# torchkge-team/torchkge

Measured on AMD Instinct MI355X. Metric: link-prediction triples scored/sec (filtered LP eval, both sides), higher is better.
Workload: dtype f32 (f16 hi/lo-split MFMA prefilter + exact f32 recheck; ranks bit-identical to f32)

## Files before the change

### torchkge_amd/csrc/lp_split_mfma.hip

```cpp
#include "kge_common.h"
#ifndef KGE_BUILD_NO_SLP
#error "build with -fno-slp-vectorize -DKGE_BUILD_NO_SLP=1 (torchkge_amd/csrc/build.py): SLP-packed v_pk_fma_f32 with a lane-crossing op_sel misreads beside co-executing MFMAs (profiles/r06/slp_bisect.txt)"
#endif

typedef _Float16 f16x8 __attribute__((ext_vector_type(8)));
typedef float f32x2 __attribute__((ext_vector_type(2)));
typedef float f32x16 __attribute__((ext_vector_type(16)));

namespace {

constexpr int TQ = 192, TC = 256;
constexpr int NT = 3;
constexpr int E_STAGE_BYTES = TC * 128;
constexpr int Q_STAGE_BYTES = TQ * 128;
constexpr int STAGE_BYTES = E_STAGE_BYTES + Q_STAGE_BYTES;
constexpr int UNC_CAP = 2048;
constexpr int GSETS = 4;
constexpr int SMEM_BYTES = 2 * STAGE_BYTES + 16 + UNC_CAP * 4 + TQ * 20 + TQ * GSETS * 12 + 16;
constexpr int SPLIT_SCALE_LOG2 = 12;

struct SplitParams {
    const char *Es, *Qs;
    int row_bytes;
    int units;
// ... 1871 lines not shown
                int qp_next, ct_next;
                item_qp_ct(it + 1, qp_next, ct_next);
                const int64_t next_q0 = (int64_t)qp_next * TQ;
                if (next_q0 != cur_q0) {
                    flush_counts(cur_q0);
                    cur_q0 = next_q0;
                    load_panel(cur_q0);
                }
            }
        }
        if (DBG && tl) {
            tsv[15] = __builtin_readcyclecounter();
            if (lane == 0) {
                unsigned long long *o = reinterpret_cast<unsigned long long *>(p.list) + ((wid >> 2) * KGE_TL_STAGES + g) * 16;
#pragma unroll
                for (int i = 0; i < 16; ++i) o[i] = tsv[i];
            }
        }
        if (++s == S) { s = 0; ++it; }
    }
#undef KGE_TS
#undef KGE_SMMA_PA
#undef KGE_SMMA_P
#undef KGE_HLOAD
#undef KGE_HWAIT
#undef KGE_SLOAD
#undef KGE_SWAIT
#undef KGE_DSR
    flush_counts(cur_q0);
}

template <bool VEC4>
__global__ __launch_bounds__(64, 2) void split_recheck_kernel(const kge_lp_desc d, const float *__restrict__ s_true,
                                                           const int32_t *__restrict__ list, int32_t cap,
                                                           const int32_t *__restrict__ list_count, int32_t *raw_count,
                                                           float *list_stat)
{
    __shared__ __attribute__((aligned(16))) float qs[64 * KGE_PS_LD];
    __shared__ __attribute__((aligned(16))) float es[64 * KGE_PS_LD];
    const int lane = threadIdx.x;
    const int n = (int)min((unsigned)*list_count, (unsigned)cap);
    if (list_stat && blockIdx.x == 0 && lane == 0) atomicAdd(list_stat, (float)n);
    const int ngroups = (n + 63) >> 6;
    for (int grp = blockIdx.x; grp < ngroups; grp += gridDim.x) {
        const int pi = grp * 64 + lane;
        const bool valid = pi < n;
        const int pj = valid ? pi : grp * 64;
        const int qi = list[2 * pj], ci = list[2 * pj + 1];
        const float sc = lp_pair_score_staged<VEC4>(d, qi, ci, qs, es);
        if (valid && !(sc >= s_true[qi])) atomicSub(&raw_count[qi], 1);
    }
}

__device__ __forceinline__ float recheck_e_segment(const float *__restrict__ T, int64_t ldt, int K, int ci,
                                                   const float *__restrict__ qrow, float *es, float acc)
{
    const int lane = threadIdx.x & 63;
    int k0 = 0;
    if (K >= KGE_PS_KC) {
        float4 e0, e1, e2, e3, e4, e5, e6, e7;
#define KGE_RR_FETCH(IT, KK)                                                                                  \
    {                                                                                                         \
        const int idx_ = lane + 64 * IT, rr_ = idx_ >> 3, pc_ = idx_ & 7;                                     \
        const int rc_ = __shfl(ci, rr_, 64);                                                                  \
        e##IT = *reinterpret_cast<const float4 *>(T + (int64_t)rc_ * ldt + (KK) + pc_ * 4);                   \
    }
#define KGE_RR_STORE(IT)                                                                                      \
    {                                                                                                         \
        const int idx_ = lane + 64 * IT, rr_ = idx_ >> 3, pc_ = idx_ & 7;                                     \
        *reinterpret_cast<float4 *>(es + rr_ * KGE_PS_LD + pc_ * 4) = e##IT;                                  \
    }
#define KGE_RR_ALL(M, ...) M(0, ##__VA_ARGS__) M(1, ##__VA_ARGS__) M(2, ##__VA_ARGS__) M(3, ##__VA_ARGS__) \
                           M(4, ##__VA_ARGS__) M(5, ##__VA_ARGS__) M(6, ##__VA_ARGS__) M(7, ##__VA_ARGS__)
        KGE_RR_ALL(KGE_RR_FETCH, 0)
        for (; k0 + KGE_PS_KC <= K; k0 += KGE_PS_KC) {
            KGE_RR_ALL(KGE_RR_STORE)
            if (k0 + 2 * KGE_PS_KC <= K) { KGE_RR_ALL(KGE_RR_FETCH, k0 + KGE_PS_KC) }
            __builtin_amdgcn_fence(__ATOMIC_SEQ_CST, "wavefront");
            acc = lp_chain_dot(qrow + k0, es + lane * KGE_PS_LD, KGE_PS_KC, acc);
            __builtin_amdgcn_fence(__ATOMIC_SEQ_CST, "wavefront");
        }
#undef KGE_RR_ALL
#undef KGE_RR_STORE
#undef KGE_RR_FETCH
    }
    for (; k0 < K; k0 += KGE_PS_KC) {
        const int kc = min(KGE_PS_KC, K - k0);
        const int pieces = kc >> 2;
        for (int idx = lane; idx < 64 * pieces; idx += 64) {
            const int rr = idx / pieces, pc = idx - rr * pieces;
            const int rc = __shfl(ci, rr, 64);
            *reinterpret_cast<float4 *>(es + rr * KGE_PS_LD + pc * 4) =
                *reinterpret_cast<const float4 *>(T + (int64_t)rc * ldt + k0 + pc * 4);
        }
        __builtin_amdgcn_fence(__ATOMIC_SEQ_CST, "wavefront");
        acc = lp_chain_dot(qrow + k0, es + lane * KGE_PS_LD, kc, acc);
        __builtin_amdgcn_fence(__ATOMIC_SEQ_CST, "wavefront");
    }
    return acc;
}

constexpr int RR_ROWS = 32, RR_PANEL = 96;

constexpr int RR_G = 4;

template <int NWV>
__global__ __launch_bounds__(64 * NWV) void split_recheck_regions_kernel(const kge_lp_desc d, const float *__restrict__ s_true,
                                                                        const int32_t *__restrict__ list, int32_t region_cap,
                                                                        const int32_t *__restrict__ region_count, int n_regions,
                                                                        int ldq, int seg_cols, int32_t *raw_count, float *list_stat,
                                                                        int32_t *list_count)
{
    extern __shared__ __attribute__((aligned(16))) float rr_smem[];
    const int tid = threadIdx.x, lane = tid & 63, wv = tid >> 6;
    float *qrows = rr_smem;
    float *es = rr_smem + RR_ROWS * ldq + wv * 64 * KGE_PS_LD;
    const int K = d.K0 + d.K1;
    int n_block = 0;
    auto stage = [&](int64_t q0, int c0, int c1) {
        const int np = (c1 - c0) >> 2;
        for (int idx = tid; idx < RR_ROWS * np; idx += 64 * NWV) {
            const int rr = idx / np, pc = idx - rr * np;
            const int64_t q = min(q0 + rr, d.B - 1);
            const int col = c0 + pc * 4;
            const float4 v = col < d.K0 ? *reinterpret_cast<const float4 *>(d.A0 + q * d.lda0 + col)
                                        : *reinterpret_cast<const float4 *>(d.A1 + q * d.lda1 + (col - d.K0));
            *reinterpret_cast<float4 *>(qrows + rr * ldq + pc * 4) = v;
        }
    };
    auto chain = [&](float acc, int ci, const float *qrow, int c0, int c1) -> float {
        if (c0 < d.K0) acc = recheck_e_segment(d.T0 + c0, d.ldt0, min(c1, d.K0) - c0, ci, qrow, es, acc);
        if (c1 > d.K0 && d.K1 > 0) {
            const int s0 = max(c0, d.K0);
            acc = recheck_e_segment(d.T1 + (s0 - d.K0), d.ldt1, c1 - s0, ci, qrow + (s0 - c0), es, acc);
        }
        return acc;
    };
    for (int reg = blockIdx.x; reg < n_regions; reg += gridDim.x) {
        const int n = (int)min((unsigned)region_count[reg], (unsigned)region_cap);
        if (n == 0) continue;
        n_block += n;
        const int64_t q0 = (int64_t)(reg / 3) * RR_PANEL + (reg % 3) * RR_ROWS;
        const int2 *ent = reinterpret_cast<const int2 *>(list) + (int64_t)reg * region_cap;
        if (K <= seg_cols) {
            __syncthreads();
            stage(q0, 0, K);
            __syncthreads();
            for (int c0 = wv * 64; c0 < n; c0 += NWV * 64) {
                const int pi = c0 + lane;
                const bool valid = pi < n;
                const int2 e = ent[valid ? pi : c0];
                const int qi = e.x, ci = e.y;
                const float acc = chain(0.0f, ci, qrows + (int)(qi - q0) * ldq, 0, K);
                const float sc = lp_epilogue_any(d, acc, qi, ci);
                if (valid && !(sc >= s_true[qi])) atomicSub(&raw_count[qi], 1);
            }
            continue;
        }
        for (int b0 = 0; b0 < n; b0 += NWV * 64 * RR_G) {
            float acc[RR_G];
            int qi[RR_G], ci[RR_G];
#pragma unroll
            for (int g = 0; g < RR_G; ++g) {
                const int c0 = b0 + (g * NWV + wv) * 64;
                const int pi = c0 + lane;
                const int2 e = ent[min(pi < n ? pi : c0, n - 1)];
                qi[g] = e.x; ci[g] = e.y; acc[g] = 0.0f;
            }
            for (int c0 = 0; c0 < K; c0 += seg_cols) {
                const int c1 = min(K, c0 + seg_cols);
                __syncthreads();
                stage(q0, c0, c1);
                __syncthreads();
#pragma unroll
                for (int g = 0; g < RR_G; ++g)
                    if (b0 + (g * NWV + wv) * 64 < n)
                        acc[g] = chain(acc[g], ci[g], qrows + (int)(qi[g] - q0) * ldq, c0, c1);
            }
#pragma unroll
            for (int g = 0; g < RR_G; ++g) {
                const int pi = b0 + (g * NWV + wv) * 64 + lane;
                if (pi < n) {
                    const float sc = lp_epilogue_any(d, acc[g], qi[g], ci[g]);
                    if (!(sc >= s_true[qi[g]])) atomicSub(&raw_count[qi[g]], 1);
                }
            }
        }
    }
    if (tid == 0 && n_block > 0) {
        if (list_stat) atomicAdd(list_stat, (float)n_block);
        if (list_count) atomicAdd(list_count, n_block);
    }
}

template <int NWAVES, bool DBG, int PM, int GS = 0, int LV = 0>
int launch_split(const SplitParams &p, int grid, hipStream_t s)
{
    auto k = lp_split_count_kernel<NWAVES, DBG, PM, GS, LV>;
    static int attr_dev[16];
    if (int e = kge_ensure_dyn_smem(reinterpret_cast<const void *>(k), SMEM_BYTES, attr_dev)) return e;
    hipLaunchKernelGGL(k, dim3(grid), dim3(64 * NWAVES), SMEM_BYTES, s, p);
    KGE_CHECK_LAUNCH();
    return 0;
}

int split_num_cus()
{
    static int n = 0;
    if (n == 0) {
        int dev = 0;
        hipDeviceProp_t prop;
        if (hipGetDevice(&dev) == hipSuccess && hipGetDeviceProperties(&prop, dev) == hipSuccess)
            n = prop.multiProcessorCount;
        if (n <= 0) n = 256;
    }
    return n;
}

inline int64_t round_up(int64_t x, int64_t m) { return (x + m - 1) / m * m; }

}

extern "C" int kge_lp_split_units(int K, int with_aug)
{
    return (int)round_up((K + (with_aug ? 1 : 0) + 15) / 16, 2);
}

extern "C" int64_t kge_lp_split_rows_padded(int64_t rows, int is_query) { return round_up(rows, is_query ? TQ : TC); }

extern "C" int kge_lp_split_rows(const float *X0, int64_t ld0, int K0, const float *X1, int64_t ld1, int K1,
                                 int64_t rows, int is_query, int aug_mode, const float *aug, float aug_mul,
                                 const float *norm2max0, const float *norm2max1, void *out, float *cell_ss,
                                 const int64_t *row_index, kge_stream_t stream)
{
    if (rows < 0 || K0 <= 0 || K1 < 0 || ld0 < K0 || (K1 > 0 && ld1 < K1) || aug_mode < 0 || aug_mode > 4)
        return KGE_EINVAL;
    if (rows == 0 && is_query) return 0;
    if ((rows > 0 && !X0) || (rows > 0 && K1 > 0 && !X1) || !out || ((aug_mode == 1 || aug_mode == 3) && rows > 0 && !aug))
        return KGE_EINVAL;
    SplitRowsParams p;
    p.X0 = X0; p.X1 = X1; p.ld0 = ld0; p.ld1 = ld1; p.K0 = K0; p.K1 = K1;
    p.rows = rows;
    p.rows_p = kge_lp_split_rows_padded(rows, is_query);
    p.aug_mode = aug_mode; p.aug = aug; p.aug_mul = aug_mul;
// ... 329 lines not shown
    int rc = kge_lp_desc_check(d);
    if (rc) return rc;
    if (d->B == 0 || d->N == 0) return 0;
    if (!s_true || !list || cap <= 0 || !list_count || !raw_count) return KGE_EINVAL;
    if (!KGE_LP_IS_MFMA(d->mode)) return KGE_EINVAL;
    const bool vec4 = kge_lp_vec4(*d);
    const int grid = split_num_cus() * kge_env_int("KGE_SPLIT_RECHECK_WAVES", 160 * 1024 / (2 * 64 * KGE_PS_LD * 4));
    if (vec4)
        hipLaunchKernelGGL(split_recheck_kernel<true>, dim3(grid), dim3(64), 0, kge_s(stream), *d, s_true, list, cap,
                           list_count, raw_count, list_stat);
    else
        hipLaunchKernelGGL(split_recheck_kernel<false>, dim3(grid), dim3(64), 0, kge_s(stream), *d, s_true, list,
                           cap, list_count, raw_count, list_stat);
    KGE_CHECK_LAUNCH();
    return 0;
}

extern "C" int kge_lp_split_regions(int64_t B)
{
    return (int)(kge_lp_split_rows_padded(B, 1) / RR_PANEL) * 3;
}

static int region_seg_cols(int K)
{
    const int max_ld = kge_env_int("KGE_REGION_MAX_BYTES", 36 * 1024) / (RR_ROWS * 4);
    const int ld_full = K + (((K >> 2) & 1) ? 0 : 4);
    if (ld_full <= max_ld) return K;
    const int seg_ld = min(max_ld, kge_env_int("KGE_REGION_SEG_BYTES", 20 * 1024) / (RR_ROWS * 4));
    int seg = ((seg_ld - 4) / 32) * 32;
    return seg < 32 ? 32 : seg;
}

extern "C" int kge_lp_split_regions_supported(const kge_lp_desc *d)
{
    if (kge_lp_desc_check(d) || !KGE_LP_IS_MFMA(d->mode) || !kge_lp_vec4(*d)) return 0;
    const int K = d->K0 + d->K1;
    if ((K + 2 + 15) / 16 > 32) return 0;
    if (region_seg_cols(K) < K && kge_env_int("KGE_REGION_SEGMENTS", 1) == 0) return 0;
    return 1;
}

extern "C" int kge_lp_split_recheck_regions(const kge_lp_desc *d, const float *s_true, const int32_t *list, int32_t cap,
                                            const int32_t *region_count, int32_t *raw_count, float *list_stat,
                                            int32_t *list_count, kge_stream_t stream)
{
    int rc = kge_lp_desc_check(d);
    if (rc) return rc;
    if (d->B == 0 || d->N == 0) return 0;
    if (!s_true || !list || cap <= 0 || !region_count || !raw_count) return KGE_EINVAL;
    if (!kge_lp_split_regions_supported(d)) return KGE_EINVAL;
    const int n_regions = kge_lp_split_regions(d->B);
    const int32_t region_cap = cap / n_regions;
    if (region_cap <= 0) return KGE_EINVAL;
    const int K = d->K0 + d->K1;
    const int seg = region_seg_cols(K);
    const int ldq = seg + (((seg >> 2) & 1) ? 0 : 4);
    const int nwv = kge_env_int("KGE_RECHECK_REGION_WAVES", 2);
    const int smem = (RR_ROWS * ldq + (nwv == 4 ? 4 : 2) * 64 * KGE_PS_LD) * 4;
    const int want = split_num_cus() * 6;
    const int grid = n_regions < want ? n_regions : want;
    static int attr2[16], attr4[16];
    if (nwv == 4) {
        auto k = split_recheck_regions_kernel<4>;
        if (int e = kge_ensure_dyn_smem(reinterpret_cast<const void *>(k), smem, attr4)) return e;
        hipLaunchKernelGGL(k, dim3(grid), dim3(256), smem, kge_s(stream), *d, s_true, list, region_cap, region_count, n_regions,
                           ldq, seg, raw_count, list_stat, list_count);
    } else {
        auto k = split_recheck_regions_kernel<2>;
        if (int e = kge_ensure_dyn_smem(reinterpret_cast<const void *>(k), smem, attr2)) return e;
        hipLaunchKernelGGL(k, dim3(grid), dim3(128), smem, kge_s(stream), *d, s_true, list, region_cap, region_count, n_regions,
                           ldq, seg, raw_count, list_stat, list_count);
    }
    KGE_CHECK_LAUNCH();
    return 0;
}

extern "C" int kge_absmax(const float *x, int64_t n, float *max_io, kge_stream_t stream)
{
    if (n < 0 || !max_io) return KGE_EINVAL;
    if (n == 0) return 0;
    if (!x) return KGE_EINVAL;
    const int64_t want = (n + 1023) / 1024;
    const int grid = (int)(want < 1024 ? want : 1024);
    hipLaunchKernelGGL(absmax_kernel, dim3(grid), dim3(256), 0, kge_s(stream), x, n, max_io);
    KGE_CHECK_LAUNCH();
    return 0;
}


extern "C" int kge_mfma_f16_selftest(void)
{
    constexpr int NT_ = 8;
    float ab[NT_][32], c[NT_], expect[NT_];
    for (int t = 0; t < NT_; ++t) { for (int k = 0; k < 32; ++k) ab[t][k] = 0.f; c[t] = 0.f; }
    auto A = [&](int t, int k) -> float & { return ab[t][k]; };
    auto Bv = [&](int t, int k) -> float & { return ab[t][16 + k]; };
    for (int k = 0; k < 16; ++k) { A(0, k) = 1.f; Bv(0, k) = 1.f; } A(0, 0) = 4096.f; Bv(0, 0) = 4096.f; expect[0] = 16777232.f;
    A(1, 0) = A(1, 1) = A(1, 2) = 1.f; Bv(1, 0) = Bv(1, 1) = Bv(1, 2) = 1.f; c[1] = 16777216.f; expect[1] = 16777220.f;
    A(2, 0) = 1.f; Bv(2, 0) = 1.f; c[2] = 16777216.f; expect[2] = 16777216.f;
    for (int k = 0; k < 16; ++k) { A(3, k) = 1.f; Bv(3, k) = 1.f; } A(3, 0) = 4096.f; Bv(3, 0) = 4096.f; A(3, 1) = 4096.f; Bv(3, 1) = -4096.f; expect[3] = 14.f;
    for (int k = 0; k < 16; ++k) { A(4, k) = 0.5f; Bv(4, k) = 1.f; } A(4, 0) = 4096.f; Bv(4, 0) = 4096.f; A(4, 1) = 4096.f; Bv(4, 1) = -4096.f; expect[4] = 4.f;
    A(5, 0) = 4096.f; Bv(5, 0) = 4096.f; A(5, 1) = 1.f; Bv(5, 1) = 1.f; A(5, 2) = 0.5f; Bv(5, 2) = 1.f; expect[5] = 16777216.f;
    A(6, 0) = 1.f; Bv(6, 0) = 1.f; A(6, 8) = 0.5f; Bv(6, 8) = 1.f; c[6] = 16777216.f; expect[6] = 16777216.f;
    A(7, 0) = 9.5367431640625e-07f; Bv(7, 0) = 1024.f; expect[7] = 0.0009765625f;
    float *d_ab = nullptr, *d_c = nullptr, *d_out = nullptr, got[NT_];
    hipError_t e = hipMalloc(&d_ab, sizeof(ab));
    if (e == hipSuccess) e = hipMalloc(&d_c, sizeof(c));
    if (e == hipSuccess) e = hipMalloc(&d_out, sizeof(got));
    if (e == hipSuccess) e = hipMemcpy(d_ab, ab, sizeof(ab), hipMemcpyHostToDevice);
    if (e == hipSuccess) e = hipMemcpy(d_c, c, sizeof(c), hipMemcpyHostToDevice);
    if (e == hipSuccess) {
        hipLaunchKernelGGL(mfma_selftest_kernel, dim3(1), dim3(64), 0, 0, d_ab, d_c, d_out, NT_);
        e = hipGetLastError();
    }
    if (e == hipSuccess) e = hipMemcpy(got, d_out, sizeof(got), hipMemcpyDeviceToHost);
    if (d_ab) (void)hipFree(d_ab);
    if (d_c) (void)hipFree(d_c);
    if (d_out) (void)hipFree(d_out);
    if (e != hipSuccess) return (int)e;
    for (int t = 0; t < NT_; ++t)
        if (got[t] != expect[t]) return 0;
    return 1;
}

// ... 122 lines not shown
```

### torchkge_amd/csrc/rank_filter.hip

```cpp
#include "kge_common.h"

int kge_lp_gemm_run(const kge_lp_desc *d, float *out, int64_t ldo, const float *s_true,
                    int32_t *raw_count, hipStream_t s);
int kge_lp_direct_count_cols(const kge_lp_desc *d, const float *s_true, int32_t *raw_count, const int64_t *rep,
                             const int32_t *col_q, int64_t n_single_p, const int32_t *members, int64_t n_multi_p,
                             hipStream_t s);
int kge_lp_direct_run(const kge_lp_desc *d, float *out, int64_t ldo, const float *s_true,
                      int32_t *raw_count, hipStream_t s);

namespace {

constexpr int RB = 256;

__device__ __forceinline__ int block_sum_i(int v, int *sh)
{
    v = wave_sum_i(v);
    const int lane = threadIdx.x & 63, w = threadIdx.x >> 6;
    __syncthreads();
    if (lane == 0) sh[w] = v;
    __syncthreads();
    int t = 0;
    for (int i = 0; i < (int)(blockDim.x >> 6); ++i) t += sh[i];
    return t;
}
// ... 351 lines not shown
        const int64_t v = b < nb ? bsum[b] : 0;
        int64_t total;
        const int64_t inc = fsub_block_scan(v, wsum, total);
        if (b < nb) bsum[b] = carry + inc - v;
        carry += total;
        __syncthreads();
    }
    if (threadIdx.x == 0) *woff_total = carry;
}
__global__ __launch_bounds__(FS_SCAN_T) void fsub_off_kernel(int64_t B, int64_t *woff, const int64_t *__restrict__ bsum)
{
    __shared__ int64_t wsum[FS_SCAN_T / 64];
    const int64_t i = (int64_t)blockIdx.x * FS_SCAN_T + threadIdx.x;
    const int64_t l = i < B ? woff[i] : 0;
    int64_t total;
    const int64_t inc = fsub_block_scan(l, wsum, total);
    if (i < B) woff[i] = bsum[blockIdx.x] + inc - l;
}

template <bool STAGED, bool VEC4, int DIRECT = 0>
__global__ __launch_bounds__(64, 2) void fsub_score_kernel(const kge_lp_desc d, const int64_t *__restrict__ seg_lo,
                                                        const int32_t *__restrict__ targets,
                                                        const int64_t *__restrict__ woff, float *fs)
{
    __shared__ __attribute__((aligned(16))) float qs[STAGED ? 64 * KGE_PS_LD : 4];
    __shared__ __attribute__((aligned(16))) float es[STAGED ? 64 * KGE_PS_LD : 4];
    const int lane = threadIdx.x;
    const int64_t W = woff[d.B];
    for (int64_t w0 = (int64_t)blockIdx.x * 64; w0 < W; w0 += (int64_t)gridDim.x * 64) {
        const int64_t w = w0 + lane;
        const bool valid = w < W;
        int64_t lo = 0, hi = d.B;
        if (valid) {
            while (lo < hi) {
                const int64_t mid = (lo + hi) >> 1;
                if (woff[mid + 1] <= w) lo = mid + 1; else hi = mid;
            }
        }
        const int64_t i = lo;
        int64_t j = 0, c = -1;
        if (valid) {
            j = seg_lo[i] + (w - woff[i]);
            c = (int64_t)targets[j] - d.c_base;
        }
        const bool ok = valid && c >= 0 && c < d.N;
        float sc;
        if constexpr (STAGED && DIRECT != 0) sc = lp_pair_score_staged_ch<VEC4, DIRECT>(d, ok ? (int)i : 0, ok ? (int)c : 0, qs, es);
        else if (STAGED) sc = lp_pair_score_staged<VEC4>(d, ok ? (int)i : 0, ok ? (int)c : 0, qs, es);
        else sc = ok ? lp_pair_score(d, i, c) : 0.f;
        if (ok) fs[j] = sc;
    }
}

constexpr int FS_SHORT = 512;
__device__ __forceinline__ void fsub_cmp(const kge_lp_desc &d, const int32_t *__restrict__ targets,
                                         const float *__restrict__ fs, int64_t j, int64_t hi, int64_t ti, float tv,
                                         int neg_inf_counts, int &sub, int &found)
{
    if (j >= hi) return;
    const int64_t cg = targets[j];
    const int64_t c = cg - d.c_base;
    if (c < 0 || c >= d.N) return;
    if (cg == ti) { found = 1; return; }
    sub += ((fs[j] >= tv) ? 1 : 0) - neg_inf_counts;
}
__device__ __forceinline__ void fsub_count_short(const kge_lp_desc &d, const float *__restrict__ s_true,
                                                 const int64_t *__restrict__ true_idx, const int64_t *__restrict__ seg_lo,
                                                 const int64_t *__restrict__ seg_hi, const int32_t *__restrict__ targets,
                                                 const float *__restrict__ fs, int skip_long, int32_t *sub_out,
                                                 int32_t *found_out, int bid, int nblk)
{
    const int lane = threadIdx.x & 63;
    const int64_t wave = (int64_t)bid * 4 + (threadIdx.x >> 6), nwaves = (int64_t)nblk * 4;
    for (int64_t i = wave; i < d.B; i += nwaves) {
        const int64_t lo = seg_lo[i], hi = seg_hi[i];
        if (skip_long && hi - lo > FS_SHORT) continue;
        int sub = 0, found = 0;
        if (hi > lo) {
            const float tv = s_true[i];
            const int64_t ti = true_idx[i];
            const int neg_inf_counts = (-INFINITY >= tv) ? 1 : 0;
            for (int64_t j0 = lo; j0 < hi; j0 += FS_SHORT) {
#pragma unroll
                for (int u = 0; u < FS_SHORT / 64; ++u)
                    fsub_cmp(d, targets, fs, j0 + u * 64 + lane, hi, ti, tv, neg_inf_counts, sub, found);
            }
            sub = wave_sum_i(sub);
            found = wave_sum_i(found);
        }
        if (lane == 0) { sub_out[i] = sub; found_out[i] = found ? 1 : 0; }
    }
}
__device__ __forceinline__ void fsub_count_long(const kge_lp_desc &d, const float *__restrict__ s_true,
                                                const int64_t *__restrict__ true_idx, const int64_t *__restrict__ seg_lo,
                                                const int64_t *__restrict__ seg_hi, const int32_t *__restrict__ targets,
                                                const float *__restrict__ fs, const int64_t *__restrict__ long_q,
                                                int64_t n_long, int32_t *sub_out, int32_t *found_out, int bid, int nblk,
                                                int *sh)
{
    for (int64_t q = bid; q < n_long; q += nblk) {
        const int64_t i = long_q[q];
        const int64_t lo = seg_lo[i], hi = seg_hi[i];
        const float tv = s_true[i];
        const int64_t ti = true_idx[i];
        const int neg_inf_counts = (-INFINITY >= tv) ? 1 : 0;
        int sub = 0, found = 0;
        for (int64_t j0 = lo; j0 < hi; j0 += 1024) {
#pragma unroll
            for (int u = 0; u < 4; ++u)
                fsub_cmp(d, targets, fs, j0 + u * 256 + threadIdx.x, hi, ti, tv, neg_inf_counts, sub, found);
        }
        sub = block_sum_i(sub, sh);
        found = block_sum_i(found, sh);
        if (threadIdx.x == 0) { sub_out[i] = sub; found_out[i] = found ? 1 : 0; }
    }
}
__global__ __launch_bounds__(256) void fsub_count_kernel(const kge_lp_desc d, const float *__restrict__ s_true,
                                                         const int64_t *__restrict__ true_idx,
                                                         const int64_t *__restrict__ seg_lo,
                                                         const int64_t *__restrict__ seg_hi,
                                                         const int32_t *__restrict__ targets,
                                                         const float *__restrict__ fs, int skip_long,
                                                         int32_t *sub_out, int32_t *found_out)
{
    fsub_count_short(d, s_true, true_idx, seg_lo, seg_hi, targets, fs, skip_long, sub_out, found_out, blockIdx.x, gridDim.x);
}
__global__ __launch_bounds__(256) void fsub_count_both_kernel(const kge_lp_desc d, const float *__restrict__ s_true,
                                                              const int64_t *__restrict__ true_idx,
                                                              const int64_t *__restrict__ seg_lo,
                                                              const int64_t *__restrict__ seg_hi,
                                                              const int32_t *__restrict__ targets,
                                                              const float *__restrict__ fs,
                                                              const int64_t *__restrict__ long_q, int64_t n_long,
                                                              int short_blocks, int32_t *sub_out, int32_t *found_out)
{
    __shared__ int sh[4];
    const int long_blocks = (int)gridDim.x - short_blocks;
    if ((int)blockIdx.x < long_blocks)
        fsub_count_long(d, s_true, true_idx, seg_lo, seg_hi, targets, fs, long_q, n_long, sub_out, found_out,
                        (int)blockIdx.x, long_blocks, sh);
    else
        fsub_count_short(d, s_true, true_idx, seg_lo, seg_hi, targets, fs, 1, sub_out, found_out,
                         (int)blockIdx.x - long_blocks, short_blocks);
}

__global__ void rank_finalize_kernel(const int32_t *__restrict__ raw, const int32_t *__restrict__ sub,
                                     const int32_t *__restrict__ found, int64_t B, int64_t *rank, int64_t *filt)
{
    for (int64_t i = (int64_t)blockIdx.x * blockDim.x + threadIdx.x; i < B; i += (int64_t)gridDim.x * blockDim.x) {
        const int64_t r = raw[i];
        rank[i] = r;
        filt[i] = found[i] ? r - sub[i] : r;
    }
}

__global__ void rank_finalize_both_kernel(const int32_t *__restrict__ raw, const int32_t *__restrict__ sub,
                                          const int32_t *__restrict__ found, int64_t B, int64_t *out, int64_t ld,
                                          int64_t off, const int64_t *__restrict__ pos,
                                          float *__restrict__ guard, float *flags, int zero_guard,
                                          int64_t *const *out_indirect)
{
    if (out_indirect) {
        out = *out_indirect;
        if (flags) flags = reinterpret_cast<float *>(out + 4 * ld);
    }
    if (flags && blockIdx.x == 0 && threadIdx.x == 0) {
        flags[0] = guard[0] + guard[1];
        flags[1] = guard[2];
        flags[2] = guard[6];
        if (zero_guard) {
#pragma unroll
            for (int j = 0; j < 8; ++j) guard[j] = 0.f;
        }
    }
    for (int64_t i = (int64_t)blockIdx.x * blockDim.x + threadIdx.x; i < 2 * B; i += (int64_t)gridDim.x * blockDim.x) {
        const bool tail = i < B;
        const int64_t j = off + (tail ? i : i - B);
        const int64_t f = pos ? pos[j] : j;
        const int64_t r = raw[i];
        out[(tail ? 1 : 0) * ld + f] = r;
        out[(tail ? 3 : 2) * ld + f] = found[i] ? r - sub[i] : r;
    }
}

__global__ __launch_bounds__(256) void lp_batched_kernel(int mode, const float *__restrict__ q, int64_t ldq,
                                                         const float *__restrict__ cand, int64_t stride_b,
                                                         int64_t stride_n, int64_t B, int64_t N, int K,
                                                         float *out, int64_t ldo)
{
    const int lane = threadIdx.x & 63;
    const int64_t wave = (int64_t)blockIdx.x * 4 + (threadIdx.x >> 6);
    const int64_t total = B * N;
    for (int64_t pidx = wave; pidx < total; pidx += (int64_t)gridDim.x * 4) {
        const int64_t i = pidx / N, c = pidx - i * N;
        const float *qq = q + i * ldq;
        const float *cc = cand + i * stride_b + c * stride_n;
// ... 383 lines not shown
                               ci, P, out);
            break;
        case KGE_LP_TORUS_EL2:
            hipLaunchKernelGGL((pair_scores_staged_kernel<true, KGE_LP_TORUS_EL2>), dim3(grid), dim3(64), 0, kge_s(stream), *d, qi,
                               ci, P, out);
            break;
        default:
            hipLaunchKernelGGL((pair_scores_staged_kernel<true, 2>), dim3(grid), dim3(64), 0, kge_s(stream), *d, qi, ci, P, out);
        }
    } else {
        hipLaunchKernelGGL(pair_scores_kernel, dim3(grid1d(P, 64)), dim3(64), 0, kge_s(stream), *d, qi, ci, P, out);
    }
    KGE_CHECK_LAUNCH();
    return 0;
}

extern "C" int kge_lp_filter_sub(const kge_lp_desc *d, const float *s_true, const int64_t *true_idx,
                                 const int64_t *seg_lo, const int64_t *seg_hi, const int32_t *targets,
                                 int32_t *sub, int32_t *found, kge_stream_t stream)
{
    int rc = kge_lp_desc_check(d);
    if (rc) return rc;
    if (d->B == 0) return 0;
    if (!s_true || !true_idx || !seg_lo || !seg_hi || !sub || !found) return KGE_EINVAL;
    if (KGE_LP_IS_MFMA(d->mode) && d->N > 0 && d->B <= INT32_MAX && d->N <= INT32_MAX) {
        const int64_t groups = (d->B + 7) / 8;
        const int grid = (int)(groups < 256 * 14 ? groups : 256 * 14);
        if (kge_lp_vec4(*d))
            hipLaunchKernelGGL(filter_sub_staged_kernel<true>, dim3(grid), dim3(64), 0, kge_s(stream), *d, s_true,
                               true_idx, seg_lo, seg_hi, targets, sub, found);
        else
            hipLaunchKernelGGL(filter_sub_staged_kernel<false>, dim3(grid), dim3(64), 0, kge_s(stream), *d, s_true,
                               true_idx, seg_lo, seg_hi, targets, sub, found);
    } else {
        hipLaunchKernelGGL(filter_sub_kernel, dim3(grid1d(d->B, 32)), dim3(256), 0, kge_s(stream), *d, s_true, true_idx,
                           seg_lo, seg_hi, targets, sub, found);
    }
    KGE_CHECK_LAUNCH();
    return 0;
}

static inline int64_t fsub_align(int64_t x) { return (x + 255) & ~(int64_t)255; }
static inline int64_t fsub_nblocks(int64_t B) { return (B + FS_SCAN_T - 1) / FS_SCAN_T; }

extern "C" int64_t kge_lp_filter_sub_ws_bytes(int64_t B, int64_t n_targets)
{
    if (B < 0 || n_targets < 0) return 0;
    return fsub_align(n_targets * 4) * 2 + fsub_align((B + 1) * 8) + fsub_align((fsub_nblocks(B) + 1) * 8);
}

static int fsub_score_and_count(const kge_lp_desc *d, const float *s_true, const int64_t *true_idx,
                                const int64_t *seg_lo, const int64_t *seg_hi, const int32_t *targets, int64_t n_pairs_max,
                                const int64_t *woff, const int64_t *long_q, int64_t n_long, float *fs, int32_t *sub,
                                int32_t *found, hipStream_t st)
{
    if (n_pairs_max > 0 && d->N > 0) {
        const int64_t groups = (n_pairs_max + 63) / 64;
        const int grid = (int)(groups < 256 * 14 ? groups : 256 * 14);
        if (KGE_LP_IS_MFMA(d->mode)) {
            if (kge_lp_vec4(*d))
                hipLaunchKernelGGL((fsub_score_kernel<true, true>), dim3(grid), dim3(64), 0, st, *d, seg_lo, targets, woff, fs);
            else
                hipLaunchKernelGGL((fsub_score_kernel<true, false>), dim3(grid), dim3(64), 0, st, *d, seg_lo, targets, woff, fs);
        } else if (!d->Wq && kge_lp_vec4(*d)) {
            switch (d->mode) {
            case KGE_LP_L1_DIRECT:
                hipLaunchKernelGGL((fsub_score_kernel<true, true, 1>), dim3(grid), dim3(64), 0, st, *d, seg_lo, targets, woff, fs);
                break;
            case KGE_LP_TORUS_L1:
                hipLaunchKernelGGL((fsub_score_kernel<true, true, KGE_LP_TORUS_L1>), dim3(grid), dim3(64), 0, st, *d, seg_lo, targets,
                                   woff, fs);
                break;
            case KGE_LP_TORUS_L2:
                hipLaunchKernelGGL((fsub_score_kernel<true, true, KGE_LP_TORUS_L2>), dim3(grid), dim3(64), 0, st, *d, seg_lo, targets,
                                   woff, fs);
                break;
            case KGE_LP_TORUS_EL2:
                hipLaunchKernelGGL((fsub_score_kernel<true, true, KGE_LP_TORUS_EL2>), dim3(grid), dim3(64), 0, st, *d, seg_lo, targets,
                                   woff, fs);
                break;
            default:
                hipLaunchKernelGGL((fsub_score_kernel<true, true, 2>), dim3(grid), dim3(64), 0, st, *d, seg_lo, targets, woff, fs);
            }
        } else {
            hipLaunchKernelGGL((fsub_score_kernel<false, false>), dim3(grid), dim3(64), 0, st, *d, seg_lo, targets, woff, fs);
        }
    }
    if (long_q && n_long > 0) {
        const int sb = grid1d(d->B, 4), lb = (int)(n_long < 256 * 16 ? n_long : 256 * 16);
        hipLaunchKernelGGL(fsub_count_both_kernel, dim3(sb + lb), dim3(256), 0, st, *d, s_true, true_idx, seg_lo, seg_hi,
                           targets, fs, long_q, n_long, sb, sub, found);
    } else {
        hipLaunchKernelGGL(fsub_count_kernel, dim3(grid1d(d->B, 4)), dim3(256), 0, st, *d, s_true, true_idx, seg_lo, seg_hi,
                           targets, fs, long_q ? 1 : 0, sub, found);
    }
    KGE_CHECK_LAUNCH();
    return 0;
}

extern "C" int kge_lp_filter_sub_grouped(const kge_lp_desc *d, const float *s_true, const int64_t *true_idx,
                                         const int64_t *seg_lo, const int64_t *seg_hi, const int32_t *targets,
                                         int64_t n_targets, int32_t *sub, int32_t *found, void *ws, int64_t ws_bytes,
                                         kge_stream_t stream)
{
    int rc = kge_lp_desc_check(d);
    if (rc) return rc;
    if (d->B == 0) return 0;
    if (!s_true || !true_idx || !seg_lo || !seg_hi || !sub || !found || n_targets < 0) return KGE_EINVAL;
    if (n_targets > 0 && (!targets || !ws || ws_bytes < kge_lp_filter_sub_ws_bytes(d->B, n_targets))) return KGE_EINVAL;
    if (d->B > INT32_MAX || d->N > INT32_MAX) return KGE_EINVAL;
    hipStream_t st = kge_s(stream);
    char *w8 = static_cast<char *>(ws);
    unsigned *claim = reinterpret_cast<unsigned *>(w8);
    float *fs = reinterpret_cast<float *>(w8 + fsub_align(n_targets * 4));
    int64_t *woff = reinterpret_cast<int64_t *>(w8 + 2 * fsub_align(n_targets * 4));
    int64_t *bsum = reinterpret_cast<int64_t *>(w8 + 2 * fsub_align(n_targets * 4) + fsub_align((d->B + 1) * 8));
    if (n_targets > 0 && d->N > 0) {
        const int nb = (int)fsub_nblocks(d->B);
        hipLaunchKernelGGL(fsub_reset_kernel, dim3(grid1d(d->B, 256)), dim3(256), 0, st, seg_lo, seg_hi, d->B, claim);
        hipLaunchKernelGGL(fsub_claim_kernel, dim3(grid1d(d->B, 256)), dim3(256), 0, st, seg_lo, seg_hi, d->B, claim);
        hipLaunchKernelGGL(fsub_len_kernel, dim3(nb), dim3(FS_SCAN_T), 0, st, seg_lo, seg_hi, d->B, claim, woff, bsum);
        hipLaunchKernelGGL(fsub_bscan_kernel, dim3(1), dim3(FS_SCAN_T), 0, st, bsum, (int64_t)nb, woff + d->B);
        hipLaunchKernelGGL(fsub_off_kernel, dim3(nb), dim3(FS_SCAN_T), 0, st, d->B, woff, bsum);
    }
    return fsub_score_and_count(d, s_true, true_idx, seg_lo, seg_hi, targets, n_targets, woff, nullptr, 0, fs, sub, found, st);
}

extern "C" int kge_lp_filter_sub_planned(const kge_lp_desc *d, const float *s_true, const int64_t *true_idx,
                                         const int64_t *seg_lo, const int64_t *seg_hi, const int32_t *targets,
                                         int64_t n_targets, const int64_t *woff, int64_t n_pairs,
                                         const int64_t *long_q, int64_t n_long, float *fs, int32_t *sub, int32_t *found,
                                         kge_stream_t stream)
{
    int rc = kge_lp_desc_check(d);
    if (rc) return rc;
    if (d->B == 0) return 0;
    if (!s_true || !true_idx || !seg_lo || !seg_hi || !sub || !found || !woff || n_targets < 0 || n_pairs < 0 || n_long < 0)
        return KGE_EINVAL;
    if (n_targets > 0 && (!targets || !fs)) return KGE_EINVAL;
    if (n_long > 0 && !long_q) return KGE_EINVAL;
    if (d->B > INT32_MAX || d->N > INT32_MAX) return KGE_EINVAL;
    return fsub_score_and_count(d, s_true, true_idx, seg_lo, seg_hi, targets, n_pairs, woff, long_q, n_long, fs, sub, found,
                                kge_s(stream));
}

extern "C" int kge_rank_finalize(const int32_t *raw, const int32_t *sub, const int32_t *found, int64_t B,
                                 int64_t *rank, int64_t *filt_rank, kge_stream_t stream)
{
    if (B < 0) return KGE_EINVAL;
    if (B == 0) return 0;
    if (!raw || !sub || !found || !rank || !filt_rank) return KGE_EINVAL;
    hipLaunchKernelGGL(rank_finalize_kernel, dim3(grid1d(B, 256)), dim3(256), 0, kge_s(stream), raw, sub, found, B,
                       rank, filt_rank);
    KGE_CHECK_LAUNCH();
    return 0;
}

extern "C" int kge_rank_finalize_both(const int32_t *raw, const int32_t *sub, const int32_t *found, int64_t B,
                                      int64_t *out, int64_t ld, int64_t off, const int64_t *pos, float *guard,
                                      float *flags, int zero_guard, int64_t *const *out_indirect, kge_stream_t stream)
{
    if (B < 0 || off < 0 || ld < off + B) return KGE_EINVAL;
    if (B == 0) return 0;
    if (!raw || !sub || !found || (!out && !out_indirect) || (flags && !guard)) return KGE_EINVAL;
    hipLaunchKernelGGL(rank_finalize_both_kernel, dim3(grid1d(2 * B, 256)), dim3(256), 0, kge_s(stream), raw, sub,
                       found, B, out, ld, off, pos, guard, flags, (flags && zero_guard) ? 1 : 0, out_indirect);
    KGE_CHECK_LAUNCH();
    return 0;
}

extern "C" int kge_lp_scores_batched(int mode, const float *q, int64_t ldq, const float *cand,
                                     int64_t stride_b, int64_t stride_n, int64_t B, int64_t N, int K,
                                     float *out, int64_t ldo, kge_stream_t stream)
{
    if (mode != KGE_LP_DOT && mode != KGE_LP_L1_DIRECT && mode != KGE_LP_L2_DIRECT && mode != KGE_LP_TORUS_L1 &&
        mode != KGE_LP_TORUS_L2 && mode != KGE_LP_TORUS_EL2)
        return KGE_EINVAL;
    if (B < 0 || N < 0 || K <= 0 || ldo < N) return KGE_EINVAL;
    if (B == 0 || N == 0) return 0;
    if (!q || !cand || !out) return KGE_EINVAL;
    hipLaunchKernelGGL(lp_batched_kernel, dim3(grid1d(B * N, 4)), dim3(256), 0, kge_s(stream), mode, q, ldq, cand,
                       stride_b, stride_n, B, N, K, out, ldo);
    KGE_CHECK_LAUNCH();
    return 0;
}

extern "C" int kge_topk_chunk(float *scores, int64_t ld, int64_t B, int64_t C, int64_t c_base, int k,
                              const int64_t *seg_lo, const int64_t *seg_hi, const int32_t *targets,
                              const int64_t *ids_in, int64_t ld_ids, int64_t *out_idx, float *out_val, int64_t ldo,
                              int64_t col_off, kge_stream_t stream)
{
    if (B < 0 || C <= 0 || ld < C || k <= 0 || col_off < 0 || ldo < col_off + k) return KGE_EINVAL;
    if (B == 0) return 0;
    if (!scores || !out_idx || !out_val) return KGE_EINVAL;
    if (targets && (!seg_lo || !seg_hi)) return KGE_EINVAL;
    if (ids_in && ld_ids < C) return KGE_EINVAL;
// ... 59 lines not shown
```

Baseline: 1366 billion.

## Balance region recheck across waves via prefix scan and pack short filter queries

The region recheck kernel no longer assigns one region per block with a shared staged query panel. It builds a windowed prefix sum of 64-pair groups across regions and has each wave binary-search its group, staging query and entity slices per wave in LDS inside the segment loop. This removes load imbalance from uneven region counts and the block-wide barriers for staging, at the cost of refetching query rows per wave. Separately, the filter-subtraction short path packs four queries per wave with 8-way unrolled loads to cut idle lanes on short segments, and the grid is sized by LDS occupancy.

Result: no change. 1360 billion (median of 4 runs) (-0.4%).

```diff
diff --git a/torchkge_amd/csrc/lp_split_mfma.hip b/torchkge_amd/csrc/lp_split_mfma.hip
--- a/torchkge_amd/csrc/lp_split_mfma.hip
+++ b/torchkge_amd/csrc/lp_split_mfma.hip
@@ -1947,144 +1947,163 @@
     }
 }
 
-__device__ __forceinline__ float recheck_e_segment(const float *__restrict__ T, int64_t ldt, int K, int ci,
-                                                   const float *__restrict__ qrow, float *es, float acc)
-{
+constexpr int RR_ROWS = 32, RR_PANEL = 96;
+constexpr int RR_WIN = 1024;
+constexpr int RR_WLDS = (64 + RR_ROWS) * KGE_PS_LD;
+
+__device__ __forceinline__ float rr_segment(const float *__restrict__ Q, int64_t lda, int64_t q0, int64_t qmax,
+                                            const float *__restrict__ T, int64_t ldt, int K, int ci, int ql, float *es,
+                                            float *qs, float acc)
+{
+    static_assert(KGE_PS_KC == 32, "the fetch / store macros below are written out for 8 float4 pieces per row");
     const int lane = threadIdx.x & 63;
+    const float *erow = es + lane * KGE_PS_LD, *qrow = qs + ql * KGE_PS_LD;
     int k0 = 0;
     if (K >= KGE_PS_KC) {
-        float4 e0, e1, e2, e3, e4, e5, e6, e7;
+        float4 e0, e1, e2, e3, e4, e5, e6, e7, a0, a1, a2, a3;
 #define KGE_RR_FETCH(IT, KK)                                                                                  \
     {                                                                                                         \
         const int idx_ = lane + 64 * IT, rr_ = idx_ >> 3, pc_ = idx_ & 7;                                     \
         const int rc_ = __shfl(ci, rr_, 64);                                                                  \
         e##IT = *reinterpret_cast<const float4 *>(T + (int64_t)rc_ * ldt + (KK) + pc_ * 4);                   \
     }
+#define KGE_RR_QFETCH(IT, KK)                                                                                 \
+    {                                                                                                         \
+        const int idx_ = lane + 64 * IT, rr_ = idx_ >> 3, pc_ = idx_ & 7;                                     \
+        a##IT = *reinterpret_cast<const float4 *>(Q + min(q0 + rr_, qmax) * lda + (KK) + pc_ * 4);            \
+    }
 #define KGE_RR_STORE(IT)                                                                                      \
     {                                                                                                         \
         const int idx_ = lane + 64 * IT, rr_ = idx_ >> 3, pc_ = idx_ & 7;                                     \
         *reinterpret_cast<float4 *>(es + rr_ * KGE_PS_LD + pc_ * 4) = e##IT;                                  \
     }
+#define KGE_RR_QSTORE(IT)                                                                                     \
+    {                                                                                                         \
+        const int idx_ = lane + 64 * IT, rr_ = idx_ >> 3, pc_ = idx_ & 7;                                     \
+        *reinterpret_cast<float4 *>(qs + rr_ * KGE_PS_LD + pc_ * 4) = a##IT;                                  \
+    }
 #define KGE_RR_ALL(M, ...) M(0, ##__VA_ARGS__) M(1, ##__VA_ARGS__) M(2, ##__VA_ARGS__) M(3, ##__VA_ARGS__) \
                            M(4, ##__VA_ARGS__) M(5, ##__VA_ARGS__) M(6, ##__VA_ARGS__) M(7, ##__VA_ARGS__)
+#define KGE_RR_QALL(M, ...) M(0, ##__VA_ARGS__) M(1, ##__VA_ARGS__) M(2, ##__VA_ARGS__) M(3, ##__VA_ARGS__)
         KGE_RR_ALL(KGE_RR_FETCH, 0)
+        KGE_RR_QALL(KGE_RR_QFETCH, 0)
         for (; k0 + KGE_PS_KC <= K; k0 += KGE_PS_KC) {
+            __builtin_amdgcn_fence(__ATOMIC_SEQ_CST, "wavefront");
             KGE_RR_ALL(KGE_RR_STORE)
-            if (k0 + 2 * KGE_PS_KC <= K) { KGE_RR_ALL(KGE_RR_FETCH, k0 + KGE_PS_KC) }
+            KGE_RR_QALL(KGE_RR_QSTORE)
+            if (k0 + 2 * KGE_PS_KC <= K) {
+                KGE_RR_ALL(KGE_RR_FETCH, k0 + KGE_PS_KC)
+                KGE_RR_QALL(KGE_RR_QFETCH, k0 + KGE_PS_KC)
+            }
             __builtin_amdgcn_fence(__ATOMIC_SEQ_CST, "wavefront");
-            acc = lp_chain_dot(qrow + k0, es + lane * KGE_PS_LD, KGE_PS_KC, acc);
-            __builtin_amdgcn_fence(__ATOMIC_SEQ_CST, "wavefront");
-        }
+            acc = lp_chain_dot(qrow, erow, KGE_PS_KC, acc);
+        }
+#undef KGE_RR_QALL
 #undef KGE_RR_ALL
+#undef KGE_RR_QSTORE
 #undef KGE_RR_STORE
+#undef KGE_RR_QFETCH
 #undef KGE_RR_FETCH
     }
-    for (; k0 < K; k0 += KGE_PS_KC) {
-        const int kc = min(KGE_PS_KC, K - k0);
-        const int pieces = kc >> 2;
+    if (k0 < K) {
+        const int kc = K - k0, pieces = kc >> 2;
+        __builtin_amdgcn_fence(__ATOMIC_SEQ_CST, "wavefront");
         for (int idx = lane; idx < 64 * pieces; idx += 64) {
             const int rr = idx / pieces, pc = idx - rr * pieces;
             const int rc = __shfl(ci, rr, 64);
             *reinterpret_cast<float4 *>(es + rr * KGE_PS_LD + pc * 4) =
                 *reinterpret_cast<const float4 *>(T + (int64_t)rc * ldt + k0 + pc * 4);
         }
+        for (int idx = lane; idx < RR_ROWS * pieces; idx += 64) {
+            const int rr = idx / pieces, pc = idx - rr * pieces;
+            *reinterpret_cast<float4 *>(qs + rr * KGE_PS_LD + pc * 4) =
+                *reinterpret_cast<const float4 *>(Q + min(q0 + rr, qmax) * lda + k0 + pc * 4);
+        }
         __builtin_amdgcn_fence(__ATOMIC_SEQ_CST, "wavefront");
-        acc = lp_chain_dot(qrow + k0, es + lane * KGE_PS_LD, kc, acc);
-        __builtin_amdgcn_fence(__ATOMIC_SEQ_CST, "wavefront");
-    }
+        acc = lp_chain_dot(qrow, erow, kc, acc);
+    }
+    __builtin_amdgcn_fence(__ATOMIC_SEQ_CST, "wavefront");
     return acc;
 }
-
-constexpr int RR_ROWS = 32, RR_PANEL = 96;
-
-constexpr int RR_G = 4;
 
 template <int NWV>
 __global__ __launch_bounds__(64 * NWV) void split_recheck_regions_kernel(const kge_lp_desc d, const float *__restrict__ s_true,
                                                                         const int32_t *__restrict__ list, int32_t region_cap,
                                                                         const int32_t *__restrict__ region_count, int n_regions,
-                                                                        int ldq, int seg_cols, int32_t *raw_count, float *list_stat,
-                                                                        int32_t *list_count)
+                                                                        int32_t *raw_count, float *list_stat, int32_t *list_count)
 {
     extern __shared__ __attribute__((aligned(16))) float rr_smem[];
+    constexpr int NT = 64 * NWV, PER = RR_WIN / NT;
+    static_assert(RR_WIN % NT == 0, "the window scan gives every thread the same number of regions");
     const int tid = threadIdx.x, lane = tid & 63, wv = tid >> 6;
-    float *qrows = rr_smem;
-    float *es = rr_smem + RR_ROWS * ldq + wv * 64 * KGE_PS_LD;
-    const int K = d.K0 + d.K1;
-    int n_block = 0;
-    auto stage = [&](int64_t q0, int c0, int c1) {
-        const int np = (c1 - c0) >> 2;
-        for (int idx = tid; idx < RR_ROWS * np; idx += 64 * NWV) {
-            const int rr = idx / np, pc = idx - rr * np;
-            const int64_t q = min(q0 + rr, d.B - 1);
-            const int col = c0 + pc * 4;
-            const float4 v = col < d.K0 ? *reinterpret_cast<const float4 *>(d.A0 + q * d.lda0 + col)
-                                        : *reinterpret_cast<const float4 *>(d.A1 + q * d.lda1 + (col - d.K0));
-            *reinterpret_cast<float4 *>(qrows + rr * ldq + pc * 4) = v;
-        }
-    };
-    auto chain = [&](float acc, int ci, const float *qrow, int c0, int c1) -> float {
-        if (c0 < d.K0) acc = recheck_e_segment(d.T0 + c0, d.ldt0, min(c1, d.K0) - c0, ci, qrow, es, acc);
-        if (c1 > d.K0 && d.K1 > 0) {
-            const int s0 = max(c0, d.K0);
-            acc = recheck_e_segment(d.T1 + (s0 - d.K0), d.ldt1, c1 - s0, ci, qrow + (s0 - c0), es, acc);
-        }
-        return acc;
-    };
-    for (int reg = blockIdx.x; reg < n_regions; reg += gridDim.x) {
-        const int n = (int)min((unsigned)region_count[reg], (unsigned)region_cap);
-        if (n == 0) continue;
-        n_block += n;
-        const int64_t q0 = (int64_t)(reg / 3) * RR_PANEL + (reg % 3) * RR_ROWS;
-        const int2 *ent = reinterpret_cast<const int2 *>(list) + (int64_t)reg * region_cap;
-        if (K <= seg_cols) {
-            __syncthreads();
-            stage(q0, 0, K);
-            __syncthreads();
-            for (int c0 = wv * 64; c0 < n; c0 += NWV * 64) {
-                const int pi = c0 + lane;
-                const bool valid = pi < n;
-                const int2 e = ent[valid ? pi : c0];
-                const int qi = e.x, ci = e.y;
-                const float acc = chain(0.0f, ci, qrows + (int)(qi - q0) * ldq, 0, K);
-                const float sc = lp_epilogue_any(d, acc, qi, ci);
-                if (valid && !(sc >= s_true[qi])) atomicSub(&raw_count[qi], 1);
-            }
-            continue;
-        }
-        for (int b0 = 0; b0 < n; b0 += NWV * 64 * RR_G) {
-            float acc[RR_G];
-            int qi[RR_G], ci[RR_G];
-#pragma unroll
-            for (int g = 0; g < RR_G; ++g) {
-                const int c0 = b0 + (g * NWV + wv) * 64;
-                const int pi = c0 + lane;
-                const int2 e = ent[min(pi < n ? pi : c0, n - 1)];
-                qi[g] = e.x; ci[g] = e.y; acc[g] = 0.0f;
-            }
-            for (int c0 = 0; c0 < K; c0 += seg_cols) {
-                const int c1 = min(K, c0 + seg_cols);
-                __syncthreads();
-                stage(q0, c0, c1);
-                __syncthreads();
-#pragma unroll
-                for (int g = 0; g < RR_G; ++g)
-                    if (b0 + (g * NWV + wv) * 64 < n)
-                        acc[g] = chain(acc[g], ci[g], qrows + (int)(qi[g] - q0) * ldq, c0, c1);
-            }
-#pragma unroll
-            for (int g = 0; g < RR_G; ++g) {
-                const int pi = b0 + (g * NWV + wv) * 64 + lane;
-                if (pi < n) {
-                    const float sc = lp_epilogue_any(d, acc[g], qi[g], ci[g]);
-                    if (!(sc >= s_true[qi[g]])) atomicSub(&raw_count[qi[g]], 1);
-                }
-            }
-        }
-    }
-    if (tid == 0 && n_block > 0) {
-        if (list_stat) atomicAdd(list_stat, (float)n_block);
-        if (list_count) atomicAdd(list_count, n_block);
+    float *es = rr_smem + wv * RR_WLDS, *qs = es + 64 * KGE_PS_LD;
+    int *gpre = reinterpret_cast<int *>(rr_smem + NWV * RR_WLDS);
+    int *wsum = gpre + RR_WIN + 1;
+    const int gw = blockIdx.x * NWV + wv, nw = gridDim.x * NWV;
+    int64_t total_pairs = 0;
+    for (int r0 = 0; r0 < n_regions; r0 += RR_WIN) {
+        int g_own = 0, p_own = 0;
+#pragma unroll
+        for (int u = 0; u < PER; ++u) {
+            const int r = r0 + tid * PER + u;
+            const int n = r < n_regions ? (int)min((unsigned)region_count[r], (unsigned)region_cap) : 0;
+            g_own += (n + 63) >> 6;
+            p_own += n;
+        }
+        int inc = g_own;
+#pragma unroll
+        for (int o = 1; o < 64; o <<= 1) {
+            const int v = __shfl_up(inc, o, 64);
+            if (lane >= o) inc += v;
+        }
+        const int p_wave = wave_sum_i(p_own);
+        __syncthreads();
+        if (lane == 63) wsum[wv] = inc;
+        if (lane == 0) wsum[NWV + wv] = p_wave;
+        __syncthreads();
+        int before = 0, G = 0, P = 0;
+#pragma unroll
+        for (int w = 0; w < NWV; ++w) {
+            const int x = wsum[w];
+            before += w < wv ? x : 0;
+            G += x;
+            P += wsum[NWV + w];
+        }
+        int run = before + inc - g_own;
+#pragma unroll
+        for (int u = 0; u < PER; ++u) {
+            const int r = r0 + tid * PER + u;
+            gpre[tid * PER + u] = run;
+            run += r < n_regions ? ((int)min((unsigned)region_count[r], (unsigned)region_cap) + 63) >> 6 : 0;
+        }
+        if (tid == 0) gpre[RR_WIN] = G;
+        total_pairs += P;
+        __syncthreads();
+        const int nr = min(RR_WIN, n_regions - r0);
+        for (int g = gw; g < G; g += nw) {
+            int lo = 0, hi = nr - 1;
+            while (lo < hi) {
+                const int mid = (lo + hi + 1) >> 1;
+                if (gpre[mid] <= g) lo = mid; else hi = mid - 1;
+            }
+            const int reg = r0 + lo;
+            const int n = (int)min((unsigned)region_count[reg], (unsigned)region_cap);
+            const int p0 = (g - gpre[lo]) * 64, pi = p0 + lane;
+            const bool valid = pi < n;
+            const int64_t q0 = (int64_t)(reg / 3) * RR_PANEL + (reg % 3) * RR_ROWS;
+            const int2 e = reinterpret_cast<const int2 *>(list)[(int64_t)reg * region_cap + (valid ? pi : p0)];
+            const int qi = e.x, ci = e.y, ql = (int)(qi - q0);
+            float acc = 0.0f;
+            for (int sg = 0; sg < (d.K1 > 0 ? 2 : 1); ++sg)
+                acc = rr_segment(sg ? d.A1 : d.A0, sg ? d.lda1 : d.lda0, q0, d.B - 1, sg ? d.T1 : d.T0, sg ? d.ldt1 : d.ldt0,
+                                 sg ? d.K1 : d.K0, ci, ql, es, qs, acc);
+            const float sc = lp_epilogue_any(d, acc, qi, ci);
+            if (valid && !(sc >= s_true[qi])) atomicSub(&raw_count[qi], 1);
+        }
+    }
+    if (blockIdx.x == 0 && tid == 0 && total_pairs > 0) {
+        if (list_stat) atomicAdd(list_stat, (float)total_pairs);
+        if (list_count) atomicAdd(list_count, (int32_t)total_pairs);
     }
 }
 
@@ -2520,24 +2539,21 @@
     const int n_regions = kge_lp_split_regions(d->B);
     const int32_t region_cap = cap / n_regions;
     if (region_cap <= 0) return KGE_EINVAL;
-    const int K = d->K0 + d->K1;
-    const int seg = region_seg_cols(K);
-    const int ldq = seg + (((seg >> 2) & 1) ? 0 : 4);
-    const int nwv = kge_env_int("KGE_RECHECK_REGION_WAVES", 2);
-    const int smem = (RR_ROWS * ldq + (nwv == 4 ? 4 : 2) * 64 * KGE_PS_LD) * 4;
-    const int want = split_num_cus() * 6;
-    const int grid = n_regions < want ? n_regions : want;
+    const int nwv = kge_env_int("KGE_RECHECK_REGION_WAVES", 2) == 4 ? 4 : 2;
+    const int smem = (nwv * RR_WLDS + RR_WIN + 1 + 2 * nwv) * 4;
+    const int per_cu = (160 * 1024) / smem;
+    const int grid = split_num_cus() * (per_cu < 1 ? 1 : per_cu);
     static int attr2[16], attr4[16];
     if (nwv == 4) {
         auto k = split_recheck_regions_kernel<4>;
         if (int e = kge_ensure_dyn_smem(reinterpret_cast<const void *>(k), smem, attr4)) return e;
         hipLaunchKernelGGL(k, dim3(grid), dim3(256), smem, kge_s(stream), *d, s_true, list, region_cap, region_count, n_regions,
-                           ldq, seg, raw_count, list_stat, list_count);
+                           raw_count, list_stat, list_count);
     } else {
         auto k = split_recheck_regions_kernel<2>;
         if (int e = kge_ensure_dyn_smem(reinterpret_cast<const void *>(k), smem, attr2)) return e;
         hipLaunchKernelGGL(k, dim3(grid), dim3(128), smem, kge_s(stream), *d, s_true, list, region_cap, region_count, n_regions,
-                           ldq, seg, raw_count, list_stat, list_count);
+                           raw_count, list_stat, list_count);
     }
     KGE_CHECK_LAUNCH();
     return 0;
diff --git a/torchkge_amd/csrc/rank_filter.hip b/torchkge_amd/csrc/rank_filter.hip
--- a/torchkge_amd/csrc/rank_filter.hip
+++ b/torchkge_amd/csrc/rank_filter.hip
@@ -427,43 +427,61 @@
     }
 }
 
-constexpr int FS_SHORT = 512;
-__device__ __forceinline__ void fsub_cmp(const kge_lp_desc &d, const int32_t *__restrict__ targets,
-                                         const float *__restrict__ fs, int64_t j, int64_t hi, int64_t ti, float tv,
-                                         int neg_inf_counts, int &sub, int &found)
-{
-    if (j >= hi) return;
-    const int64_t cg = targets[j];
-    const int64_t c = cg - d.c_base;
-    if (c < 0 || c >= d.N) return;
-    if (cg == ti) { found = 1; return; }
-    sub += ((fs[j] >= tv) ? 1 : 0) - neg_inf_counts;
-}
+constexpr int FS_SHORT = 512, FS_U = 8;
+__device__ __forceinline__ void fsub_pass(const kge_lp_desc &d, const int32_t *__restrict__ targets,
+                                          const float *__restrict__ fs, int64_t j, int64_t stride, int64_t hi, int64_t ti,
+                                          float tv, int neg_inf_counts, int &sub, int &found)
+{
+    int32_t tg[FS_U];
+    float f[FS_U];
+#pragma unroll
+    for (int u = 0; u < FS_U; ++u) {
+        const int64_t jj = j + u * stride;
+        tg[u] = jj < hi ? targets[jj] : 0;
+        f[u] = jj < hi ? fs[jj] : 0.0f;
+    }
+#pragma unroll
+    for (int u = 0; u < FS_U; ++u) {
+        if (j + u * stride >= hi) continue;
+        const int64_t cg = tg[u];
+        const int64_t c = cg - d.c_base;
+        if (c < 0 || c >= d.N) continue;
+        if (cg == ti) { found = 1; continue; }
+        sub += ((f[u] >= tv) ? 1 : 0) - neg_inf_counts;
+    }
+}
+template <int QPW>
 __device__ __forceinline__ void fsub_count_short(const kge_lp_desc &d, const float *__restrict__ s_true,
                                                  const int64_t *__restrict__ true_idx, const int64_t *__restrict__ seg_lo,
                                                  const int64_t *__restrict__ seg_hi, const int32_t *__restrict__ targets,
                                                  const float *__restrict__ fs, int skip_long, int32_t *sub_out,
                                                  int32_t *found_out, int bid, int nblk)
 {
-    const int lane = threadIdx.x & 63;
+    constexpr int LPQ = 64 / QPW;
+    const int lane = threadIdx.x & 63, ql = lane / LPQ, sl = lane % LPQ;
     const int64_t wave = (int64_t)bid * 4 + (threadIdx.x >> 6), nwaves = (int64_t)nblk * 4;
-    for (int64_t i = wave; i < d.B; i += nwaves) {
-        const int64_t lo = seg_lo[i], hi = seg_hi[i];
-        if (skip_long && hi - lo > FS_SHORT) continue;
+    for (int64_t i0 = wave * QPW; i0 < d.B; i0 += nwaves * QPW) {
+        const int64_t i = i0 + ql;
         int sub = 0, found = 0;
-        if (hi > lo) {
+        bool mine = i < d.B;
+        int64_t lo = 0, hi = 0;
+        if (mine) {
+            lo = seg_lo[i]; hi = seg_hi[i];
+            if (skip_long && hi - lo > FS_SHORT) mine = false;
+        }
+        if (mine && hi > lo) {
             const float tv = s_true[i];
             const int64_t ti = true_idx[i];
             const int neg_inf_counts = (-INFINITY >= tv) ? 1 : 0;
-            for (int64_t j0 = lo; j0 < hi; j0 += FS_SHORT) {
-#pragma unroll
-                for (int u = 0; u < FS_SHORT / 64; ++u)
-                    fsub_cmp(d, targets, fs, j0 + u * 64 + lane, hi, ti, tv, neg_inf_counts, sub, found);
-            }
-            sub = wave_sum_i(sub);
-            found = wave_sum_i(found);
-        }
-        if (lane == 0) { sub_out[i] = sub; found_out[i] = found ? 1 : 0; }
+            for (int64_t j0 = lo; j0 < hi; j0 += LPQ * FS_U)
+                fsub_pass(d, targets, fs, j0 + sl, LPQ, hi, ti, tv, neg_inf_counts, sub, found);
+        }
+#pragma unroll
+        for (int o = LPQ / 2; o > 0; o >>= 1) {
+            sub += __shfl_xor(sub, o, 64);
+            found += __shfl_xor(found, o, 64);
+        }
+        if (mine && sl == 0) { sub_out[i] = sub; found_out[i] = found ? 1 : 0; }
     }
 }
 __device__ __forceinline__ void fsub_count_long(const kge_lp_desc &d, const float *__restrict__ s_true,
@@ -480,16 +498,14 @@
         const int64_t ti = true_idx[i];
         const int neg_inf_counts = (-INFINITY >= tv) ? 1 : 0;
         int sub = 0, found = 0;
-        for (int64_t j0 = lo; j0 < hi; j0 += 1024) {
-#pragma unroll
-            for (int u = 0; u < 4; ++u)
-                fsub_cmp(d, targets, fs, j0 + u * 256 + threadIdx.x, hi, ti, tv, neg_inf_counts, sub, found);
-        }
+        for (int64_t j0 = lo; j0 < hi; j0 += 256 * FS_U)
+            fsub_pass(d, targets, fs, j0 + threadIdx.x, 256, hi, ti, tv, neg_inf_counts, sub, found);
         sub = block_sum_i(sub, sh);
         found = block_sum_i(found, sh);
         if (threadIdx.x == 0) { sub_out[i] = sub; found_out[i] = found ? 1 : 0; }
     }
 }
+template <int QPW>
 __global__ __launch_bounds__(256) void fsub_count_kernel(const kge_lp_desc d, const float *__restrict__ s_true,
                                                          const int64_t *__restrict__ true_idx,
                                                          const int64_t *__restrict__ seg_lo,
@@ -498,8 +514,10 @@
                                                          const float *__restrict__ fs, int skip_long,
                                                          int32_t *sub_out, int32_t *found_out)
 {
-    fsub_count_short(d, s_true, true_idx, seg_lo, seg_hi, targets, fs, skip_long, sub_out, found_out, blockIdx.x, gridDim.x);
-}
+    fsub_count_short<QPW>(d, s_true, true_idx, seg_lo, seg_hi, targets, fs, skip_long, sub_out, found_out, blockIdx.x,
+                          gridDim.x);
+}
+constexpr int FS_QPW = 4;
 __global__ __launch_bounds__(256) void fsub_count_both_kernel(const kge_lp_desc d, const float *__restrict__ s_true,
                                                               const int64_t *__restrict__ true_idx,
                                                               const int64_t *__restrict__ seg_lo,
@@ -515,8 +533,8 @@
         fsub_count_long(d, s_true, true_idx, seg_lo, seg_hi, targets, fs, long_q, n_long, sub_out, found_out,
                         (int)blockIdx.x, long_blocks, sh);
     else
-        fsub_count_short(d, s_true, true_idx, seg_lo, seg_hi, targets, fs, 1, sub_out, found_out,
-                         (int)blockIdx.x - long_blocks, short_blocks);
+        fsub_count_short<FS_QPW>(d, s_true, true_idx, seg_lo, seg_hi, targets, fs, 1, sub_out, found_out,
+                                 (int)blockIdx.x - long_blocks, short_blocks);
 }
 
 __global__ void rank_finalize_kernel(const int32_t *__restrict__ raw, const int32_t *__restrict__ sub,
@@ -1006,7 +1024,7 @@
 static int fsub_score_and_count(const kge_lp_desc *d, const float *s_true, const int64_t *true_idx,
                                 const int64_t *seg_lo, const int64_t *seg_hi, const int32_t *targets, int64_t n_pairs_max,
                                 const int64_t *woff, const int64_t *long_q, int64_t n_long, float *fs, int32_t *sub,
-                                int32_t *found, hipStream_t st)
+                                int32_t *found, bool planned, hipStream_t st)
 {
     if (n_pairs_max > 0 && d->N > 0) {
         const int64_t groups = (n_pairs_max + 63) / 64;
@@ -1041,12 +1059,15 @@
         }
     }
     if (long_q && n_long > 0) {
-        const int sb = grid1d(d->B, 4), lb = (int)(n_long < 256 * 16 ? n_long : 256 * 16);
+        const int sb = grid1d(d->B, 4 * FS_QPW), lb = (int)(n_long < 256 * 16 ? n_long : 256 * 16);
         hipLaunchKernelGGL(fsub_count_both_kernel, dim3(sb + lb), dim3(256), 0, st, *d, s_true, true_idx, seg_lo, seg_hi,
                            targets, fs, long_q, n_long, sb, sub, found);
+    } else if (planned) {
+        hipLaunchKernelGGL(fsub_count_kernel<FS_QPW>, dim3(grid1d(d->B, 4 * FS_QPW)), dim3(256), 0, st, *d, s_true, true_idx,
+                           seg_lo, seg_hi, targets, fs, long_q ? 1 : 0, sub, found);
     } else {
-        hipLaunchKernelGGL(fsub_count_kernel, dim3(grid1d(d->B, 4)), dim3(256), 0, st, *d, s_true, true_idx, seg_lo, seg_hi,
-                           targets, fs, long_q ? 1 : 0, sub, found);
+        hipLaunchKernelGGL(fsub_count_kernel<1>, dim3(grid1d(d->B, 4)), dim3(256), 0, st, *d, s_true, true_idx, seg_lo, seg_hi,
+                           targets, fs, 0, sub, found);
     }
     KGE_CHECK_LAUNCH();
     return 0;
@@ -1077,7 +1098,8 @@
         hipLaunchKernelGGL(fsub_bscan_kernel, dim3(1), dim3(FS_SCAN_T), 0, st, bsum, (int64_t)nb, woff + d->B);
         hipLaunchKernelGGL(fsub_off_kernel, dim3(nb), dim3(FS_SCAN_T), 0, st, d->B, woff, bsum);
     }
-    return fsub_score_and_count(d, s_true, true_idx, seg_lo, seg_hi, targets, n_targets, woff, nullptr, 0, fs, sub, found, st);
+    return fsub_score_and_count(d, s_true, true_idx, seg_lo, seg_hi, targets, n_targets, woff, nullptr, 0, fs, sub, found, false,
+                                st);
 }
 
 extern "C" int kge_lp_filter_sub_planned(const kge_lp_desc *d, const float *s_true, const int64_t *true_idx,
@@ -1095,7 +1117,7 @@
     if (n_long > 0 && !long_q) return KGE_EINVAL;
     if (d->B > INT32_MAX || d->N > INT32_MAX) return KGE_EINVAL;
     return fsub_score_and_count(d, s_true, true_idx, seg_lo, seg_hi, targets, n_pairs, woff, long_q, n_long, fs, sub, found,
-                                kge_s(stream));
+                                true, kge_s(stream));
 }
 
 extern "C" int kge_rank_finalize(const int32_t *raw, const int32_t *sub, const int32_t *found, int64_t B,
```
